# REXJJ/high-fidelity-pointcloud-fusion

Measured on AMD Instinct MI355X. Metric: Mpts/s fused into 1 mm voxel grid, higher is better.
Workload: dtype f64

## Files before the change

### high-fidelity-pointcloud-fusion_amd/csrc/hfpf.hip

```cpp
#include <hip/hip_runtime.h>

#include <cstring>

#include <rocprim/rocprim.hpp>

#include <dlfcn.h>
#include <sched.h>
#include <sys/mman.h>

#if !defined(__HIP_DEVICE_COMPILE__)
#include <emmintrin.h>
#endif
#include <algorithm>
#include <atomic>
#include <condition_variable>
#include <cmath>
#include <cstdarg>
#include <cstdio>
#include <cstdlib>
#include <cstring>
#include <mutex>
#include <string>
#include <thread>
#include <vector>
// ... 109 lines not shown
                    spins = 0;
                }
            }
            if (stop_.load(std::memory_order_acquire)) return;
            seen = g;
            part(i);
            remaining_.fetch_sub(1, std::memory_order_acq_rel);
        }
    }
    std::vector<std::thread> th_;
    std::mutex m_;
    std::condition_variable cv_;
    std::atomic<uint64_t> gen_{0};
    std::atomic<int> remaining_{0}, sleepers_{0};
    std::atomic<bool> stop_{false};
    char* dst_ = nullptr;
    const char* src_ = nullptr;
    size_t bytes_ = 0;
};

constexpr int kStageSlots = 8;
constexpr size_t kXferChunk = 16u << 20;
#ifndef HFPF_PROBE_FRAMES
#define HFPF_PROBE_FRAMES 8
#endif
constexpr int kProbeFrames = HFPF_PROBE_FRAMES;
constexpr int kFrameSlots = 8;

struct DepthSpec {
    uint32_t width, height, depth_f32, depth_step, color_bpp, color_bgr, color_step;
    float cx, cy, sx, sy, unit;
    uint32_t color_off;
    size_t depth_bytes() const { return (size_t)(height - 1) * depth_step + (size_t)width * (depth_f32 ? 4u : 2u); }
    size_t color_bytes() const { return color_bpp ? (size_t)(height - 1) * color_step + (size_t)width * color_bpp : 0; }
};
static_assert(sizeof(DepthSpec) == 13 * 4, "DepthSpec is compared bytewise");

DepthLayout depth_layout(const DepthSpec& d, const void* dev_color, uint64_t color_stride)
{
    return DepthLayout{d.color_bpp ? (const uint8_t*)dev_color : nullptr, color_stride, d.width, d.depth_step, d.color_step, d.depth_f32,
                       d.color_bpp, d.color_bgr, d.cx, d.cy, d.sx, d.sy, d.unit};
}

struct Knobs {
    int copy_streams = 2;
    bool update_cells = true;
    int host_batch = 4;
    int upd_shape_forced = -1;
    bool trace_shape = false;
    bool bin_spare = true;
    bool stream_replay = true;
    float bin_slack = 2.0f;
    bool clean_small_nowait = true;
    float test_bin_scale = 1.f;
    bool test_table_skip = false;
    bool mailbox = true;
    int test_dev_tile = kDevTileDefault;
    int stage_threads = 0;
};

struct Session {
    bool dirty = false;
    uint64_t n_linked[kLogRegions] = {0};
    uint64_t gate_done = 0;
    bool pend_valid = false;
    uint64_t direct_linked = 0;
    bool normals_possible = false;
    uint32_t next_frame_id = 0;
    bool poisoned = false;
    std::string poison_msg;
    bool bin_have_hist = false;
    bool bin_from_probe = false;
    double bin_prev_points = 0;
    uint64_t n_bricks_known = 0;
    uint64_t n_bricks_before = 0;
    unsigned long long upd_miss_seen = 0, upd_member_seen = 0;
    unsigned long long pub_seq = 0;
    uint32_t pend_n = 0, pend_first = 0;
    uint32_t pend_pts = 0;
    uint32_t pend_lay[5] = {0, 0, 0, 0, 0};
    bool pend_depth = false;
    DepthSpec pend_ds{};
    double pend_pose[kFrameSlots * 12] = {0};
    uint64_t occ_exported = 0;
    uint64_t frames_exported = 0, frames_seen = 0;
};

using EventPairs = std::vector<std::pair<hipEvent_t, hipEvent_t>>;

}

struct hfpf_handle {
    std::mutex mtx;
    std::string err;

    hfpf_config cfg;
    GridParams g;
    Knobs knobs;
    bool binned = false;
    int integrate_grid = 1536;
    size_t dir_entries = 0;
    uint64_t n_slots = 0;
    uint64_t max_touched = 0;

    Session ss;
    uint64_t frames_integrated = 0;
    uint64_t clean_passes = 0;
    uint32_t launch_seq = 0;
    bool upd_wide = false;
    bool epoch_used = false;
    unsigned long long mbox_seq = 0;
    int stage_next = 0, fslot_next = 0;

    Tables t;
    hipStream_t stream = nullptr;
    hipStream_t copy_stream = nullptr;
    hipStream_t copy_more[3] = {nullptr, nullptr, nullptr};
    std::vector<void*> allocs;
    uint64_t device_bytes = 0;
    unsigned long long* h_ctr = nullptr;
    unsigned long long* h_log_ctr = nullptr;
    unsigned long long* mbox = nullptr;
    DevBuf pend_a, pend_b;
    StageSlot stage[kStageSlots];
    FrameSlot fslot[kFrameSlots];
    void* ring_d = nullptr;
    size_t ring_cap = 0;
    hipEvent_t busy_ev = nullptr;
    bool busy_pending = false;
    void* xfer_pin[2] = {nullptr, nullptr};
    hipEvent_t xfer_ev[2] = {nullptr, nullptr};
    StagePool* stage_pool = nullptr;
    DevBuf sort_tmp, keys_a, keys_b, vals_a, vals_b, rows_dev, probe_a, probe_b, probe_c, probe_d, probe_e, probe_f;
    DevBuf zbuf, render_pose, render_out;
    DevBuf track_in, track_acc;
    DevBuf query_in, query_out;
    DevBuf mesh_cube, mesh_corner, mesh_kdata, mesh_cdata, mesh_out, mesh_ctr;
    DevBuf comp_index, comp_rows, comp_recs, comp_out;
    DevBuf dev_mesh, dev_tri, dev_bins, dev_pairs, dev_out;
    DevBuf ray_in, ray_out, ray_map;
    DevBuf snap_stage, snap_err;
    uint64_t bin_pool = 0;
    DevBuf bin_pt_buf, bin_rgb_buf, bin_sums;
    DevBuf ovf_pt_buf, ovf_aux_buf;
    bool dist_on = false;
    int rank = 0, world = 1;
    void* rccl_lib = nullptr;
    void* comm = nullptr;
    uint64_t ex_cap_records = 0;
    DevBuf ex_send, ex_recv, ex_counts, stats_total;
    unsigned long long* h_counts = nullptr;

    bool timing = false;
    bool timing_detail = false;
    std::vector<hipEvent_t> ev_detail;
    std::vector<uint8_t> ev_detail_ran;
    double t_detail_ms[3] = {0, 0, 0};
    uint64_t n_detail[3] = {0, 0, 0};
    EventPairs ev_pending, ev_pending_clean;
    EventPairs ev_pending_ray;
// ... 150 lines not shown
    h->h_ctr[C_REPLAY_MEMBER] = replayed;
    unsigned long long upd_tested = 0, upd_member = 0;
    for (int r = 0; r < kLogRegions; r++) {
        upd_tested += h->h_log_ctr[r * 16 + 2];
        upd_member += h->h_log_ctr[r * 16 + 3];
    }
    h->h_ctr[C_DEP_TESTED] += upd_tested;
    h->h_ctr[C_DEP_MEMBER] += upd_member;
    unsigned long long single = 0;
    for (int r = 0; r < kLogRegions; r++) single += h->h_log_ctr[r * 16 + 4];
    h->h_ctr[C_TOUCHED_SINGLE] = single;
    {
        const uint64_t nbk = std::min<uint64_t>(h->h_ctr[C_BRICKS], h->t.max_bricks);
        if (nbk != h->ss.n_bricks_known) h->ss.n_bricks_before = h->ss.n_bricks_known;
        h->ss.n_bricks_known = nbk;
    }
    return HFPF_OK;
}

int check_device_errors(hfpf_handle* h)
{
    const unsigned long long e = h->h_ctr[C_ERR];
    if (!e) return HFPF_OK;
    std::string what;
    if (e & E_BRICKS) what += " brick pool (max_bricks)";
    if (e & E_LOG) what += " point log (max_log_points)";
    if (e & E_OCC) what += " occupied list (max_normals*4)";
    if (e & E_NORMALS) what += " normal records (max_normals)";
    if (e & E_REG) what += " registrations (max_normals*7)";
    if (e & E_DEP) what += " dependant table";
    if (e & E_SPIN) what += " brick-claim spin bound";
    if (e & E_DEPCNT) what += " more than 65535 dependants on one cell";
    if (e & E_FRAME) what += " frame id >= max_frames";
    if (e & E_OVF) what += " integrate overflow list";
    if (e & E_CHAIN) what += " point-log chain / run record out of range (internal)";
    return fail(h, HFPF_ERR_CAPACITY, "device pool overflow:%s", what.c_str());
}

float stat_scale_for(double bound) { return (float)std::ldexp(1.0, 26 - (int)std::floor(std::log2(bound))); }

Knobs read_knobs()
{
    Knobs k;
    if (const char* cs = getenv("HFPF_COPY_STREAMS")) k.copy_streams = std::max(1, std::min(atoi(cs), 4));
    const char* uf = getenv("HFPF_UPDATE_FORM");
    k.update_cells = !(uf && uf[0] == 'p');
    if (const char* hb = getenv("HFPF_HOST_BATCH")) k.host_batch = std::max(1, std::min(atoi(hb), kFrameSlots));
    if (const char* us = getenv("HFPF_UPD_SHAPE")) k.upd_shape_forced = std::max(0, std::min(atoi(us), 1));
    if (const char* tr = getenv("HFPF_TRACE_SHAPE")) k.trace_shape = tr[0] != '0';
    if (const char* sp = getenv("HFPF_BIN_SPARE")) k.bin_spare = sp[0] != '0';
    if (const char* sr = getenv("HFPF_STREAM_REPLAY")) k.stream_replay = sr[0] != '0';
    if (const char* bs = getenv("HFPF_BIN_SLACK")) k.bin_slack = std::max(1.0f, std::min(4.0f, (float)atof(bs)));
    if (const char* nw = getenv("HFPF_CLEAN_NOWAIT")) k.clean_small_nowait = nw[0] != '0';
    if (const char* bs = getenv("HFPF_TEST_BIN_SCALE")) k.test_bin_scale = std::max(0.f, std::min(1.f, (float)atof(bs)));
    const char* ts = getenv("HFPF_TEST_TABLE_SKIP");
    k.test_table_skip = ts && ts[0] == '1';
    if (const char* dt = getenv("HFPF_TEST_DEV_TILE")) k.test_dev_tile = std::max(8, std::min(atoi(dt), kDevTileMax));
    const char* mb = getenv("HFPF_MAILBOX");
    k.mailbox = !mb || mb[0] != '0';
    int cores = (int)std::thread::hardware_concurrency();
    cpu_set_t set;
    if (sched_getaffinity(0, sizeof set, &set) == 0) cores = std::min(cores > 0 ? cores : 1 << 20, CPU_COUNT(&set));
    const char* st = getenv("HFPF_STAGE_THREADS");
    k.stage_threads = st ? std::max(0, std::min(atoi(st), 15)) : std::max(0, std::min(7, cores / 2 - 1));
    return k;
}

int setup_params(hfpf_handle* h)
{
    const hfpf_config& c = h->cfg;
    GridParams& g = h->g;
    if (!(c.resolution > 0.f)) return fail(h, HFPF_ERR_BAD_CONFIG, "resolution must be > 0");
    for (int a = 0; a < 3; a++)
        if (!(c.bbox[2 * a + 1] > c.bbox[2 * a])) return fail(h, HFPF_ERR_BAD_CONFIG, "bounding_box axis %d: max <= min", a);
    if (c.k != 2) return fail(h, HFPF_ERR_BAD_CONFIG, "k must be 2 (the reference probes exactly 125 neighbours, OccupancyGrid.hpp:334)");
    if (c.K < 0 || c.K > 16) return fail(h, HFPF_ERR_BAD_CONFIG, "K out of range [0,16]");
    if (!(c.cylinder_radius > 0) || !(c.ball_radius > 0)) return fail(h, HFPF_ERR_BAD_CONFIG, "radii must be > 0");
    g.res = (double)c.resolution;
    g.inv_res = 1.0 / g.res;
    for (int a = 0; a < 3; a++) {
        g.min[a] = c.bbox[2 * a];
        g.max[a] = c.bbox[2 * a + 1];
        const double d = (g.max[a] - g.min[a]) / g.res;
        if (!(d < 2097151.0)) return fail(h, HFPF_ERR_BAD_CONFIG, "axis %d: more than 2^21 cells", a);
        g.dim[a] = (int32_t)d;
        g.bdim[a] = (g.dim[a] + 1 + 7) / 8;
    }
    {
        auto bits_for = [](int32_t dim) {
            uint32_t b = 1;
            while ((1ll << b) <= (long long)dim) b++;
            return b;
        };
        g.key_sy = bits_for(g.dim[2]);
        g.key_sx = g.key_sy + bits_for(g.dim[1]);
        g.key_bits = g.key_sx + bits_for(g.dim[0]);
    }
    g.zclip_min = c.z_clip_min;
    g.zclip_max = c.z_clip_max;
    {
        auto float_at_or_above = [](double m) {
            float f = (float)m;
            if ((double)f < m) f = nextafterf(f, INFINITY);
            return f;
        };
        auto float_at_or_below = [](double m) {
// ... 92 lines not shown
    int rc;
#define ALLOC(field, count, ...)                                         \
    if ((rc = dev_alloc(h, &t.field, (count), ##__VA_ARGS__)) != HFPF_OK) return rc;
    ALLOC(dir, h->dir_entries, 0, false);
    ALLOC(brick_lin, t.max_bricks + 1);
    ALLOC(info, h->n_slots, 0, false);
    ALLOC(first_frame, h->n_slots, 0, false);
    ALLOC(buf_head, h->n_slots * kChains, 0, false);
    ALLOC(stat_id, h->n_slots, 0, false);
    ALLOC(pre_dep, h->n_slots, 0, false);
    ALLOC(dep_tmp, h->n_slots, 0, false);
    ALLOC(occ_mask, (t.max_bricks + 1) * 8, 0, false);
    ALLOC(log_pt, t.max_log + 1, 0, false);
    if (c.flags & HFPF_FLAG_FUSE_COLOR) { ALLOC(log_rgb, t.max_log + 1, 0, false); }
    ALLOC(occ_list, t.max_occ, 0, false);
    ALLOC(nv_key, t.max_normals + 1, 0, false);
    ALLOC(nv_slot, t.max_normals + 1, 0, false);
    ALLOC(nv_c, 3 * (t.max_normals + 1), 0, false);
    ALLOC(nv_n, 3 * (t.max_normals + 1), 0, false);
    ALLOC(stats, (t.max_normals + 1) * kStatWords, 0, false);
    t.color = (c.flags & HFPF_FLAG_FUSE_COLOR) ? 1u : 0u;
    t.test_table_skip = h->knobs.test_table_skip ? 1u : 0u;
    ALLOC(nd_mask, (t.max_bricks + 1) * 8 * 2, 0, false);
    ALLOC(reg_occ, t.max_reg, 0, false);
    ALLOC(dep, t.max_dep + t.max_normals + 1, 0, false);
    t.nv_line = reinterpret_cast<float4*>(t.dep + t.max_dep);
    ALLOC(prereg_list, t.max_reg, 0, false);
    ALLOC(touched_list, h->max_touched, 0, false);
    ALLOC(run_start, t.max_bricks + 2, 0, false);
    ALLOC(run_len, t.max_bricks + 2, 0, false);
    ALLOC(run_cnt, t.max_bricks + 2);
    ALLOC(cand_key, t.max_occ, 0, false);
    ALLOC(frame_vp, 3 * t.max_frames);
    ALLOC(frame_list, t.max_frames, 0, false);
    ALLOC(ctr, C_COUNT);
    ALLOC(log_ctr, kLogRegions * 16);
    ALLOC(bin_fill, 2 * (t.max_bricks + 2));
    ALLOC(bin_off, 2 * (t.max_bricks + 2));
    ALLOC(bin_capb, 2 * (t.max_bricks + 2));
    h->binned = (c.flags & HFPF_FLAG_DIRECT_UPDATE) == 0;
#undef ALLOC
    t.log_region_cap = t.max_log / kLogRegions;
    t.ent_base = t.dep;
    t.ent_dep_first = 0;
    t.ent_nv_first = t.max_dep;
    return reset_state(h);
}

#ifndef HFPF_SORT_BLOCK_ITEMS
#define HFPF_SORT_BLOCK_ITEMS 4
#endif
using sort_config = rocprim::radix_sort_config<rocprim::default_config, rocprim::merge_sort_config<512, 1024, HFPF_SORT_BLOCK_ITEMS>, rocprim::default_config>;

int sort_keys_u64(hfpf_handle* h, uint64_t* in, uint64_t* out, uint64_t n, unsigned bits = 0)
{
    const unsigned kb = bits ? bits : h->g.key_bits;
    size_t bytes = 0;
    HIPCHK(h, rocprim::radix_sort_keys<sort_config>(nullptr, bytes, in, out, (size_t)n, 0, kb, h->stream));
    int rc = scratch(h, h->sort_tmp, bytes);
    if (rc) return rc;
    bytes = h->sort_tmp.bytes;
    HIPCHK(h, rocprim::radix_sort_keys<sort_config>(h->sort_tmp.p, bytes, in, out, (size_t)n, 0, kb, h->stream));
    return HFPF_OK;
}

int sort_keys_u32(hfpf_handle* h, uint32_t* in, uint32_t* out, uint64_t n, unsigned bits = 32)
{
    size_t bytes = 0;
    HIPCHK(h, rocprim::radix_sort_keys<sort_config>(nullptr, bytes, in, out, (size_t)n, 0, bits, h->stream));
    int rc = scratch(h, h->sort_tmp, bytes);
    if (rc) return rc;
    bytes = h->sort_tmp.bytes;
    HIPCHK(h, rocprim::radix_sort_keys<sort_config>(h->sort_tmp.p, bytes, in, out, (size_t)n, 0, bits, h->stream));
    return HFPF_OK;
}

int sort_pairs_u64(hfpf_handle* h, uint64_t* kin, uint64_t* kout, uint32_t* vin, uint32_t* vout, uint64_t n, unsigned bits = 0)
{
    const unsigned kb = bits ? bits : h->g.key_bits;
    size_t bytes = 0;
    HIPCHK(h, rocprim::radix_sort_pairs<sort_config>(nullptr, bytes, kin, kout, vin, vout, (size_t)n, 0, kb, h->stream));
    int rc = scratch(h, h->sort_tmp, bytes);
    if (rc) return rc;
    bytes = h->sort_tmp.bytes;
    HIPCHK(h, rocprim::radix_sort_pairs<sort_config>(h->sort_tmp.p, bytes, kin, kout, vin, vout, (size_t)n, 0, kb, h->stream));
    return HFPF_OK;
}

int acquire_stage(hfpf_handle* h, uint32_t n_frames, StageSlot** out)
{
    StageSlot& s = h->stage[h->stage_next];
    h->stage_next = (h->stage_next + 1) % kStageSlots;
    if (s.pending) {
        HIPCHK(h, hipEventSynchronize(s.done));
        s.pending = false;
    }
    if (!s.done) HIPCHK(h, hipEventCreateWithFlags(&s.done, hipEventDisableTiming));
    if (s.cap < n_frames) {
        if (s.h_pose) {
            HIPCHK(h, hipHostFree(s.h_pose));
            HIPCHK(h, hipFree(s.d_pose));
            s.h_pose = nullptr, s.d_pose = nullptr, s.cap = 0;
        }
        const uint32_t cap = std::max<uint32_t>(n_frames, 64);
        const size_t bytes = (size_t)cap * (12 * sizeof(double) + sizeof(uint32_t));
        HIPCHK(h, hipHostMalloc((void**)&s.h_pose, bytes, hipHostMallocDefault));
        HIPCHK(h, hipMalloc((void**)&s.d_pose, bytes));
        s.cap = cap;
    }
    s.h_ids = reinterpret_cast<uint32_t*>(s.h_pose + 12 * (size_t)n_frames);
    s.d_ids = reinterpret_cast<uint32_t*>(s.d_pose + 12 * (size_t)n_frames);
    *out = &s;
    return HFPF_OK;
}

int pick_update_shape(hfpf_handle* h, double points, uint32_t nb)
{
    (void)points;
    (void)nb;
    if (h->knobs.upd_shape_forced >= 0) return h->knobs.upd_shape_forced;
    const unsigned long long miss = h->h_ctr[C_TABLE_MISS], member = h->h_ctr[C_DEP_MEMBER] + h->h_ctr[C_REPLAY_MEMBER];
    if (h->knobs.trace_shape)
        fprintf(stderr, "hfpf: update shape window: %llu table misses, %llu members (%llu of them replayed so far), %s\n", miss - std::min(miss, h->ss.upd_miss_seen),
                member - std::min(member, h->ss.upd_member_seen), h->h_ctr[C_REPLAY_MEMBER], h->upd_wide ? "wide" : "dense");
    if (!h->upd_wide && miss > h->ss.upd_miss_seen && (miss - h->ss.upd_miss_seen) * 500ull > member - std::min(member, h->ss.upd_member_seen)) h->upd_wide = true;
    h->ss.upd_miss_seen = miss;
    h->ss.upd_member_seen = member;
    return h->upd_wide ? 1 : 0;
// ... 3736 lines not shown
    PROBE_DOWN(proj_out, h->probe_d, n * 12);
    PROBE_DOWN(dist_out, h->probe_e, n * 8);
    PROBE_DOWN(member_out, h->probe_f, n);
    HIPCHK(h, hipStreamSynchronize(h->stream));
    return HFPF_OK;
}

int hfpf_probe_depth(hfpf_handle* h, const hfpf_depth_image* desc, const void* depth, const void* color, float* xyz_out, uint32_t* rgb_out)
{
    if (!h || !xyz_out || !rgb_out) return HFPF_ERR_BAD_ARG;
    std::lock_guard<std::mutex> lk(h->mtx);
    HIPCHK(h, hipSetDevice(h->cfg.device));
    DepthSpec ds;
    int rc = depth_spec(h, desc, depth, color, &ds);
    if (rc) return rc;
    const uint32_t n = ds.width * ds.height;
    PROBE_UP(h->probe_a, depth, ds.depth_bytes());
    if (ds.color_bpp) {
        PROBE_UP(h->probe_b, color, ds.color_bytes());
    }
    if ((rc = scratch(h, h->probe_c, (size_t)n * 12))) return rc;
    if ((rc = scratch(h, h->probe_d, (size_t)n * 4))) return rc;
    hipLaunchKernelGGL(k_probe_depth, dim3(blocks_for(n, 256)), dim3(256), 0, h->stream, depth_layout(ds, h->probe_b.p, 0), (const uint8_t*)h->probe_a.p, n,
                       (float*)h->probe_c.p, (uint32_t*)h->probe_d.p);
    HIPCHK(h, hipGetLastError());
    PROBE_DOWN(xyz_out, h->probe_c, (size_t)n * 12);
    PROBE_DOWN(rgb_out, h->probe_d, (size_t)n * 4);
    HIPCHK(h, hipStreamSynchronize(h->stream));
    return HFPF_OK;
}

int hfpf_probe_trig(hfpf_handle* h, uint64_t n, const float* y, const float* x, float* atan2_out, float* cos_out, float* sin_out)
{
    if (!h || !y || !x || !atan2_out || !cos_out || !sin_out) return HFPF_ERR_BAD_ARG;
    std::lock_guard<std::mutex> lk(h->mtx);
    HIPCHK(h, hipSetDevice(h->cfg.device));
    if (n == 0) return HFPF_OK;
    int rc;
    PROBE_UP(h->probe_a, y, n * 4);
    PROBE_UP(h->probe_b, x, n * 4);
    if ((rc = scratch(h, h->probe_c, n * 4))) return rc;
    if ((rc = scratch(h, h->probe_d, n * 4))) return rc;
    if ((rc = scratch(h, h->probe_e, n * 4))) return rc;
    hipLaunchKernelGGL(k_probe_trig, dim3(blocks_for(n, 256)), dim3(256), 0, h->stream, n, (const float*)h->probe_a.p, (const float*)h->probe_b.p,
                       (float*)h->probe_c.p, (float*)h->probe_d.p, (float*)h->probe_e.p);
    HIPCHK(h, hipGetLastError());
    PROBE_DOWN(atan2_out, h->probe_c, n * 4);
    PROBE_DOWN(cos_out, h->probe_d, n * 4);
    PROBE_DOWN(sin_out, h->probe_e, n * 4);
    HIPCHK(h, hipStreamSynchronize(h->stream));
    return HFPF_OK;
}

}
```

### high-fidelity-pointcloud-fusion_amd/csrc/kernels.hpp

```cpp
#pragma once
#include <type_traits>

#include "stats.hpp"

namespace hfpf {

typedef float vf4 __attribute__((ext_vector_type(4)));

struct FrameLayout {
    uint32_t point_step, off_x, off_y, off_z, off_rgb;
};

struct DepthLayout {
    const uint8_t* color;
    uint64_t color_stride;
    uint32_t width, depth_step, color_step;
    uint32_t depth_f32;
    uint32_t color_bpp;
    uint32_t color_bgr;
    float cx, cy, sx, sy, unit;
};

template <bool WANT_RGB>
__device__ __forceinline__ vf4 depth_fetch(const uint8_t* __restrict__ dimg, const uint8_t* __restrict__ cimg, const DepthLayout& L, uint32_t i)
// ... 3591 lines not shown
            for (uint32_t e = threadIdx.x; e < nt * 12u; e += 256u) s_tri[e] = ((const double*)recs)[(uint64_t)s_idx[e / 12u] * 12u + e % 12u];
            __syncthreads();
            if (have) {
                for (uint32_t j = 0; j < nt; j++) {
                    double Q[3];
                    uint32_t region;
                    const double dd = dev_closest(P, &s_tri[j * 12u], Q, region);
                    if (dd <= md2 && (!found || dd < best)) {
                        const double* N = &s_tri[j * 12u + 9u];
                        const double rr[3] = {P[0] - Q[0], P[1] - Q[1], P[2] - Q[2]};
                        found = true, best = dd, btri = s_idx[j], breg = region, neg = dev_dot(N, rr) < 0.0;
                        bq[0] = Q[0], bq[1] = Q[1], bq[2] = Q[2];
                    }
                }
            }
        }
        if (have) {
            Deviation d;
            if (found) {
                d.distance = (float)sqrt(best);
                d.signed_distance = neg ? -d.distance : d.distance;
                d.tri = btri, d.flags = kDevFound | breg;
                d.q[0] = (float)bq[0], d.q[1] = (float)bq[1], d.q[2] = (float)bq[2];
                const double w = (double)d.distance;
                n_found++;
                n_neg += d.signed_distance < 0.f ? 1u : 0u;
                max_bits = max(max_bits, __float_as_uint(d.distance));
                sum_abs += llrint(w * 0x1p30);
                sum_sq += llrint((w * w) * 0x1p30);
            } else {
                d.distance = d.signed_distance = d.q[0] = d.q[1] = d.q[2] = __uint_as_float(0x7FC00000u);
                d.tri = 0xFFFFFFFFu, d.flags = 0u;
            }
            d.reserved = 0u;
            out[row] = d;
        }
    }
    for (int o = 32; o > 0; o >>= 1) {
        n_found += __shfl_down(n_found, o);
        n_neg += __shfl_down(n_neg, o);
        sum_abs += __shfl_down(sum_abs, o);
        sum_sq += __shfl_down(sum_sq, o);
        max_bits = max(max_bits, __shfl_down(max_bits, o));
    }
    if ((threadIdx.x & 63u) == 0 && n_found) {
        atomicAdd(&sum->n_found, n_found);
        if (n_neg) atomicAdd(&sum->n_negative, n_neg);
        atomicAdd((unsigned long long*)&sum->sum_abs_q30, (unsigned long long)sum_abs);
        atomicAdd((unsigned long long*)&sum->sum_sq_q30, (unsigned long long)sum_sq);
        atomicMax(&sum->max_abs_bits, max_bits);
    }
}

}
```

### high-fidelity-pointcloud-fusion_amd/python/hfpf.py

```python
import ctypes as C
import os
import subprocess

import numpy as np

_HERE = os.path.dirname(os.path.abspath(__file__))
PKG_DIR = os.path.dirname(_HERE)
CSRC_DIR = os.path.join(PKG_DIR, "csrc")
LIB_PATH = os.environ.get("HFPF_LIB") or os.path.join(CSRC_DIR, "libhfpf.so")

FLAG_FUSE_COLOR = 1
FLAG_PCL_SHIFTED_COV = 2
FLAG_DIRECT_UPDATE = 4
STATUS = {0: "OK", -1: "BAD_CONFIG", -2: "BAD_ARG", -3: "CAPACITY", -4: "HIP", -5: "STATE", -6: "IO", -7: "DIST"}


class HfpfError(RuntimeError):
    def __init__(self, code, msg):
        super().__init__("hfpf status %d (%s): %s" % (code, STATUS.get(code, "?"), msg))
        self.code = code


class Config(C.Structure):
    _fields_ = [
        ("struct_size", C.c_uint32),
        ("resolution", C.c_float),
        ("bbox", C.c_double * 6),
        ("k", C.c_int32),
        ("K", C.c_int32),
        ("gate", C.c_int32),
        ("cylinder_radius", C.c_double),
        ("ball_radius", C.c_double),
        ("z_clip_min", C.c_double),
        ("z_clip_max", C.c_double),
        ("device", C.c_int32),
        ("flags", C.c_uint32),
        ("max_bricks", C.c_uint64),
        ("max_log_points", C.c_uint64),
        ("max_normals", C.c_uint64),
        ("max_frames", C.c_uint64),
        ("frame_width", C.c_uint32),
        ("reserved0", C.c_uint32),
        ("max_call_points", C.c_uint64),
    ]


class ExtractOpts(C.Structure):
    _fields_ = [("struct_size", C.c_uint32), ("classify_threshold", C.c_int32), ("min_count", C.c_double),
                ("paint_white", C.c_int32), ("reserved0", C.c_int32)]


class Counters(C.Structure):
    _fields_ = [(n, C.c_uint64) for n in (
        "points_presented", "points_zclip_pass", "points_in_bbox", "points_buffered", "dep_pairs_tested",
        "dep_pairs_member", "voxels_occupied", "voxels_with_normal", "bricks_allocated", "registrations",
        "dep_entries", "frames_integrated", "clean_passes", "device_bytes", "replay_members", "points_direct", "table_misses", "update_extra_rounds")]


ROW_DTYPE = np.dtype(
    [
        ("ix", "<i4"), ("iy", "<i4"), ("iz", "<i4"), ("count", "<u4"),
        ("x", "<f4"), ("y", "<f4"), ("z", "<f4"),
        ("nx", "<f4"), ("ny", "<f4"), ("nz", "<f4"),
        ("sdx", "<f4"), ("sdy", "<f4"), ("sdz", "<f4"),
        ("mean_dist", "<f4"), ("sd_dist", "<f4"), ("rgb", "<u4"),
    ]
)

EXPORTS = [
    "hfpf_default_config", "hfpf_abi_version", "hfpf_create", "hfpf_destroy", "hfpf_last_error", "hfpf_get_dims",
    "hfpf_integrate", "hfpf_integrate_pinned", "hfpf_host_alloc", "hfpf_host_free", "hfpf_integrate_device", "hfpf_is_dirty", "hfpf_clean", "hfpf_extract", "hfpf_extract_filtered", "hfpf_free_rows",
    "hfpf_write_pcd", "hfpf_write_meta_csv", "hfpf_write_pcd_xyzrgb", "hfpf_write_pcd_binary", "hfpf_clear", "hfpf_sync", "hfpf_get_counters", "hfpf_get_occupied",
    "hfpf_device_alloc", "hfpf_device_free", "hfpf_device_upload", "hfpf_kernel_timing", "hfpf_get_kernel_time",
    "hfpf_probe_points", "hfpf_probe_normals", "hfpf_probe_project", "hfpf_probe_trig",
    "hfpf_dist_unique_id", "hfpf_dist_init", "hfpf_dist_info", "hfpf_dist_disable", "hfpf_epoch_export", "hfpf_epoch_import", "hfpf_stats_export",
    "hfpf_extract_with_stats", "hfpf_device_download", "hfpf_device_copy", "hfpf_epoch_import_gathered",
    "hfpf_integrate_depth", "hfpf_integrate_depth_pinned", "hfpf_integrate_depth_device", "hfpf_probe_depth",
    "hfpf_render", "hfpf_render_device",
    "hfpf_track_depth", "hfpf_track_depth_device", "hfpf_track",
    "hfpf_query", "hfpf_query_device", "hfpf_query_depth",
    "hfpf_extract_mesh", "hfpf_extract_mesh_device", "hfpf_free_mesh", "hfpf_write_ply", "hfpf_check_mesh_opts",
    "hfpf_check_component_opts", "hfpf_extract_components", "hfpf_extract_components_device", "hfpf_free_components",
    "hfpf_check_deviation_opts", "hfpf_compare_mesh", "hfpf_compare_mesh_device", "hfpf_free_deviation", "hfpf_read_ply",
    "hfpf_check_raycast_opts", "hfpf_raycast", "hfpf_raycast_device", "hfpf_raycast_view", "hfpf_raycast_view_device",
    "hfpf_snapshot", "hfpf_free_snapshot", "hfpf_restore", "hfpf_save", "hfpf_load", "hfpf_snapshot_info", "hfpf_config_from_snapshot",
]

DEPTH_U16, DEPTH_F32 = 1, 2
COLOR_NONE, COLOR_RGB8, COLOR_BGR8, COLOR_RGBA8, COLOR_BGRA8 = 0, 1, 2, 3, 4
COLOR_BPP = {COLOR_NONE: 0, COLOR_RGB8: 3, COLOR_BGR8: 3, COLOR_RGBA8: 4, COLOR_BGRA8: 4}


class DepthImage(C.Structure):
    _fields_ = [("struct_size", C.c_uint32), ("width", C.c_uint32), ("height", C.c_uint32), ("depth_format", C.c_uint32),
                ("depth_step", C.c_uint32), ("depth_scale", C.c_float), ("fx", C.c_double), ("fy", C.c_double),
                ("cx", C.c_double), ("cy", C.c_double), ("color_format", C.c_uint32), ("color_step", C.c_uint32),
                ("reserved", C.c_uint64)]


def depth_desc(width, height, depth_format, depth_step, K, color_format=COLOR_NONE, color_step=0, depth_scale=0.001):
    d = DepthImage()
    d.struct_size = C.sizeof(DepthImage)
    d.width, d.height, d.depth_format, d.depth_step = width, height, depth_format, depth_step
    d.depth_scale = depth_scale
    d.fx, d.fy, d.cx, d.cy = (float(k) for k in K)
    d.color_format, d.color_step = color_format, color_step
    return d


def _image_desc(depth, K, color, color_format, depth_scale):
    if depth.ndim != 2 or depth.dtype not in (np.uint16, np.float32) or depth.strides[1] != depth.itemsize:
        raise ValueError("depth must be a 2-D uint16 or float32 image with contiguous rows")
    fmt = DEPTH_U16 if depth.dtype == np.uint16 else DEPTH_F32
    H, W = depth.shape
    cstep = 0
    if color is None:
        color_format = COLOR_NONE
    else:
        if color.dtype != np.uint8 or color.ndim != 3 or color.shape[:2] != depth.shape or color.strides[2] != 1 or color.strides[1] != color.shape[2]:
            raise ValueError("color must be a HxWx3 or HxWx4 uint8 image with contiguous rows, the size of the depth image")
        if color_format is None:
            color_format = COLOR_RGB8 if color.shape[2] == 3 else COLOR_RGBA8
        if COLOR_BPP.get(color_format) != color.shape[2]:
            raise ValueError("color_format %r does not match a %d-channel image" % (color_format, color.shape[2]))
        cstep = color.strides[0]
    return depth_desc(W, H, fmt, depth.strides[0], K, color_format, cstep, depth_scale)

RENDER_CULL_BACKFACES = 1
RENDER_WORLD_NORMALS = 2
RENDER_PLANES = (("depth", np.float32, 1), ("normal", np.float32, 3), ("rgb", np.uint32, 1), ("count", np.uint32, 1), ("voxel", np.int32, 3))
# ... 304 lines not shown
    L = C.CDLL(LIB_PATH)
    vp, u32, u64, i32 = C.c_void_p, C.c_uint32, C.c_uint64, C.c_int32
    L.hfpf_default_config.argtypes = [C.POINTER(Config)]
    L.hfpf_default_config.restype = None
    L.hfpf_abi_version.restype = C.c_int
    L.hfpf_create.argtypes = [C.POINTER(Config), C.POINTER(vp)]
    L.hfpf_destroy.argtypes = [vp]
    L.hfpf_last_error.argtypes = [vp]
    L.hfpf_last_error.restype = C.c_char_p
    L.hfpf_get_dims.argtypes = [vp, C.POINTER(i32), C.POINTER(C.c_double)]
    L.hfpf_integrate.argtypes = [vp, vp, u32, u32, u32, u32, u32, u32, vp]
    L.hfpf_integrate_device.argtypes = [vp, vp, u32, u64, u32, u32, u32, u32, u32, u32, vp, vp]
    L.hfpf_integrate_pinned.argtypes = [vp, vp, u32, u32, u32, u32, u32, u32, vp]
    L.hfpf_host_alloc.argtypes = [vp, u64, C.POINTER(vp)]
    L.hfpf_host_free.argtypes = [vp, vp]
    L.hfpf_is_dirty.argtypes = [vp]
    L.hfpf_clean.argtypes = [vp]
    L.hfpf_extract.argtypes = [vp, C.POINTER(vp), C.POINTER(u64)]
    L.hfpf_extract_filtered.argtypes = [vp, C.POINTER(ExtractOpts), C.POINTER(vp), C.POINTER(u64)]
    L.hfpf_free_rows.argtypes = [vp]
    L.hfpf_free_rows.restype = None
    L.hfpf_write_pcd.argtypes = [vp, u64, C.c_char_p]
    L.hfpf_write_meta_csv.argtypes = [vp, u64, C.c_char_p]
    L.hfpf_write_pcd_xyzrgb.argtypes = [vp, u64, C.c_char_p, u32, i32, i32]
    L.hfpf_write_pcd_binary.argtypes = [vp, u64, C.c_char_p]
    L.hfpf_clear.argtypes = [vp]
    L.hfpf_sync.argtypes = [vp]
    L.hfpf_get_counters.argtypes = [vp, C.POINTER(Counters)]
    L.hfpf_get_occupied.argtypes = [vp, vp, u64, C.POINTER(u64)]
    L.hfpf_device_alloc.argtypes = [vp, u64, C.POINTER(vp)]
    L.hfpf_device_free.argtypes = [vp, vp]
    L.hfpf_device_upload.argtypes = [vp, vp, vp, u64]
    L.hfpf_kernel_timing.argtypes = [vp, C.c_int]
    L.hfpf_get_kernel_time.argtypes = [vp, C.c_int, C.POINTER(C.c_double), C.POINTER(u64)]
    L.hfpf_probe_points.argtypes = [vp, vp, vp, u64, vp, vp, vp]
    L.hfpf_probe_normals.argtypes = [vp, u64, vp, vp, vp, vp, vp]
    L.hfpf_probe_project.argtypes = [vp, u64, vp, vp, vp, vp, vp, vp]
    L.hfpf_probe_trig.argtypes = [vp, u64, vp, vp, vp, vp, vp]
    L.hfpf_dist_unique_id.argtypes = [vp]
    L.hfpf_dist_init.argtypes = [vp, C.c_int, C.c_int, vp]
    L.hfpf_dist_disable.argtypes = [vp]
    L.hfpf_dist_info.argtypes = [vp, C.POINTER(i32), C.POINTER(i32)]
    L.hfpf_epoch_export.argtypes = [vp, C.POINTER(vp), C.POINTER(u64)]
    L.hfpf_epoch_import.argtypes = [vp, vp, u64]
    L.hfpf_stats_export.argtypes = [vp, C.POINTER(vp), C.POINTER(u64), C.POINTER(vp), C.POINTER(u64)]
    L.hfpf_extract_with_stats.argtypes = [vp, vp, vp, C.POINTER(vp), C.POINTER(u64)]
    L.hfpf_device_download.argtypes = [vp, vp, vp, u64]
    L.hfpf_device_copy.argtypes = [vp, vp, vp, u64]
    L.hfpf_epoch_import_gathered.argtypes = [vp, vp, u64, i32, i32, vp]
    L.hfpf_integrate_depth.argtypes = [vp, C.POINTER(DepthImage), vp, vp, vp]
    L.hfpf_integrate_depth_pinned.argtypes = [vp, C.POINTER(DepthImage), vp, vp, vp]
    L.hfpf_integrate_depth_device.argtypes = [vp, C.POINTER(DepthImage), vp, u64, vp, u64, u32, vp, vp]
    L.hfpf_probe_depth.argtypes = [vp, C.POINTER(DepthImage), vp, vp, vp, vp]
    L.hfpf_render.argtypes = [vp, C.POINTER(RenderOpts), vp, C.POINTER(RenderPlanes)]
    L.hfpf_render_device.argtypes = [vp, C.POINTER(RenderOpts), u32, vp, C.POINTER(RenderPlanes)]
    L.hfpf_track_depth.argtypes = [vp, C.POINTER(TrackOpts), C.POINTER(DepthImage), vp, vp, C.POINTER(TrackResult)]
    L.hfpf_track_depth_device.argtypes = [vp, C.POINTER(TrackOpts), C.POINTER(DepthImage), vp, vp, C.POINTER(TrackResult)]
    L.hfpf_track.argtypes = [vp, C.POINTER(TrackOpts), vp, u32, u32, u32, u32, u32, vp, C.POINTER(TrackResult)]
    L.hfpf_query.argtypes = [vp, C.POINTER(QueryOpts), vp, u32, u32, u32, u32, u32, vp, vp, vp]
    L.hfpf_query_device.argtypes = [vp, C.POINTER(QueryOpts), vp, u32, u32, u32, u32, u32, vp, vp, vp]
    L.hfpf_query_depth.argtypes = [vp, C.POINTER(QueryOpts), C.POINTER(DepthImage), vp, vp, vp, vp]
    L.hfpf_extract_mesh.argtypes = [vp, C.POINTER(MeshOpts), C.POINTER(vp), C.POINTER(u64), C.POINTER(vp), C.POINTER(u64)]
    L.hfpf_extract_mesh_device.argtypes = [vp, C.POINTER(MeshOpts), C.POINTER(vp), C.POINTER(u64), C.POINTER(vp), C.POINTER(u64)]
    L.hfpf_free_mesh.argtypes = [vp, vp]
    L.hfpf_free_mesh.restype = None
    L.hfpf_write_ply.argtypes = [vp, u64, vp, u64, C.c_char_p]
    L.hfpf_check_mesh_opts.argtypes = [C.POINTER(MeshOpts)]
    L.hfpf_check_component_opts.argtypes = [C.POINTER(ComponentOpts)]
    for fn in (L.hfpf_extract_components, L.hfpf_extract_components_device):
        fn.argtypes = [vp, C.POINTER(ComponentOpts), C.POINTER(vp), C.POINTER(vp), C.POINTER(u64), C.POINTER(vp), C.POINTER(u64)]
    L.hfpf_free_components.argtypes = [vp, vp, vp]
    L.hfpf_free_components.restype = None
    L.hfpf_check_deviation_opts.argtypes = [C.POINTER(DeviationOpts)]
    for fn in (L.hfpf_compare_mesh, L.hfpf_compare_mesh_device):
        fn.argtypes = [vp, C.POINTER(DeviationOpts), vp, u64, u32, vp, u64, vp, C.POINTER(vp), C.POINTER(vp), C.POINTER(u64),
                       C.POINTER(DeviationSummary)]
    L.hfpf_free_deviation.argtypes = [vp, vp]
    L.hfpf_free_deviation.restype = None
    L.hfpf_read_ply.argtypes = [C.c_char_p, C.POINTER(vp), C.POINTER(u64), C.POINTER(vp), C.POINTER(u64)]
    dbl = C.c_double
    L.hfpf_check_raycast_opts.argtypes = [C.POINTER(RaycastOpts)]
    L.hfpf_raycast.argtypes = [vp, C.POINTER(RaycastOpts), vp, u64, vp, vp]
    L.hfpf_raycast_device.argtypes = [vp, C.POINTER(RaycastOpts), vp, u64, vp, vp]
    L.hfpf_raycast_view.argtypes = [vp, C.POINTER(RaycastOpts), u32, u32, dbl, dbl, dbl, dbl, vp, vp]
    L.hfpf_raycast_view_device.argtypes = [vp, C.POINTER(RaycastOpts), u32, u32, dbl, dbl, dbl, dbl, u32, vp, vp]
    L.hfpf_snapshot.argtypes = [vp, C.POINTER(vp), C.POINTER(u64)]
    L.hfpf_free_snapshot.argtypes = [vp]
    L.hfpf_free_snapshot.restype = None
    L.hfpf_restore.argtypes = [vp, vp, u64]
    L.hfpf_save.argtypes = [vp, C.c_char_p]
    L.hfpf_load.argtypes = [vp, C.c_char_p]
    L.hfpf_snapshot_info.argtypes = [vp, u64, C.POINTER(SnapshotInfo)]
    L.hfpf_config_from_snapshot.argtypes = [C.POINTER(SnapshotInfo), C.POINTER(Config)]
    _lib = L
    return L


def _p(a):
    return a.ctypes.data_as(C.c_void_p)


def default_config():
    c = Config()
    lib().hfpf_default_config(C.byref(c))
    return c

# ... 502 lines not shown
        return ms.value, n.value

    def probe_points(self, pose, xyz):
        pose = np.ascontiguousarray(pose, dtype=np.float64).reshape(12)
        xyz = np.ascontiguousarray(xyz, dtype=np.float32).reshape(-1, 3)
        n = xyz.shape[0]
        q = np.zeros((n, 3), np.float32)
        idx = np.zeros((n, 3), np.int32)
        flags = np.zeros(n, np.uint8)
        self._chk(lib().hfpf_probe_points(self._h, _p(pose), _p(xyz), n, _p(q), _p(idx), _p(flags)))
        return q, idx, flags

    def probe_normals(self, cells, occ, vps):
        cells = np.ascontiguousarray(cells, dtype=np.int32).reshape(-1, 3)
        n = cells.shape[0]
        occ = np.ascontiguousarray(occ, dtype=np.uint8).reshape(n, 125)
        vps = np.ascontiguousarray(vps, dtype=np.float32).reshape(n, 3)
        normals = np.zeros((n, 3), np.float32)
        totals = np.zeros(n, np.int32)
        self._chk(lib().hfpf_probe_normals(self._h, n, _p(cells), _p(occ), _p(vps), _p(normals), _p(totals)))
        return normals, totals

    def probe_project(self, pts, centres, normals):
        pts = np.ascontiguousarray(pts, dtype=np.float32).reshape(-1, 3)
        n = pts.shape[0]
        centres = np.ascontiguousarray(centres, dtype=np.float32).reshape(n, 3)
        normals = np.ascontiguousarray(normals, dtype=np.float32).reshape(n, 3)
        proj = np.zeros((n, 3), np.float32)
        dist = np.zeros(n, np.float64)
        member = np.zeros(n, np.uint8)
        self._chk(lib().hfpf_probe_project(self._h, n, _p(pts), _p(centres), _p(normals), _p(proj), _p(dist), _p(member)))
        self.last_member_kernel_form = (member & 2) != 0
        self.last_hoisted_division_same = (member & 4) != 0
        return proj, dist, (member & 1) != 0

    def probe_depth(self, depth, K, color=None, color_format=None, depth_scale=0.001):
        d = _image_desc(depth, K, color, color_format, depth_scale)
        n = d.width * d.height
        xyz = np.zeros((n, 3), np.float32)
        rgb = np.zeros(n, np.uint32)
        self._chk(lib().hfpf_probe_depth(self._h, C.byref(d), C.c_void_p(depth.ctypes.data),
                                         C.c_void_p(color.ctypes.data) if color is not None else None, _p(xyz), _p(rgb)))
        return xyz, rgb

    def probe_trig(self, y, x):
        y = np.ascontiguousarray(y, dtype=np.float32)
        x = np.ascontiguousarray(x, dtype=np.float32)
        a = np.zeros_like(x)
        c = np.zeros_like(x)
        s = np.zeros_like(x)
        self._chk(lib().hfpf_probe_trig(self._h, x.size, _p(y), _p(x), _p(a), _p(c), _p(s)))
        return a, c, s


def dist_unique_id():
    buf = (C.c_char * 128)()
    rc = lib().hfpf_dist_unique_id(buf)
    if rc != 0:
        raise HfpfError(rc, lib().hfpf_last_error(None).decode())
    return bytes(buf)


def write_pcd(rows, path):
    rows = np.ascontiguousarray(rows, dtype=ROW_DTYPE)
    rc = lib().hfpf_write_pcd(_p(rows), rows.size, os.fsencode(path))
    if rc != 0:
        raise HfpfError(rc, "write_pcd(%s)" % path)


def write_meta_csv(rows, path):
    rows = np.ascontiguousarray(rows, dtype=ROW_DTYPE)
    rc = lib().hfpf_write_meta_csv(_p(rows), rows.size, os.fsencode(path))
    if rc != 0:
        raise HfpfError(rc, "write_meta_csv(%s)" % path)


def write_pcd_xyzrgb(rows, path, min_count=0, classify_threshold=-1, white=True):
    rows = np.ascontiguousarray(rows, dtype=ROW_DTYPE)
    rc = lib().hfpf_write_pcd_xyzrgb(_p(rows), rows.size, os.fsencode(path), min_count, classify_threshold, 1 if white else 0)
    if rc != 0:
        raise HfpfError(rc, "write_pcd_xyzrgb(%s)" % path)


def write_pcd_binary(rows, path):
    rows = np.ascontiguousarray(rows, dtype=ROW_DTYPE)
    rc = lib().hfpf_write_pcd_binary(_p(rows), rows.size, os.fsencode(path))
    if rc != 0:
        raise HfpfError(rc, "write_pcd_binary(%s)" % path)
```

### include/hfpf_probe.h

```cpp
#ifndef HFPF_PROBE_H
#define HFPF_PROBE_H
#include "hfpf.h"
#ifdef __cplusplus
extern "C" {
#endif

int hfpf_probe_points(hfpf_handle* h, const double pose_3x4[12], const float* xyz, uint64_t n, float* q_out,
                      int32_t* idx_out, uint8_t* flags_out);
int hfpf_probe_normals(hfpf_handle* h, uint64_t n, const int32_t* cells, const uint8_t* occ, const float* vps,
                       float* normals_out, int32_t* totals_out);
int hfpf_probe_project(hfpf_handle* h, uint64_t n, const float* pts, const float* centres, const float* normals,
                       float* proj_out, double* dist_out, uint8_t* member_out);
int hfpf_probe_depth(hfpf_handle* h, const hfpf_depth_image* desc, const void* depth, const void* color, float* xyz_out,
                     uint32_t* rgb_out);
int hfpf_probe_trig(hfpf_handle* h, uint64_t n, const float* y, const float* x, float* atan2_out, float* cos_out,
                    float* sin_out);

#ifdef __cplusplus
}
#endif
#endif
```

Measured before the change: 28240.

## Add single-block LDS radix sort for small key arrays

Adds a one-workgroup, 1024-thread radix sort kernel, using 5-bit digits with shared-memory counters. sort_keys_u32 and sort_keys_u64 now route arrays of up to about 31.7K keys to it instead of rocprim's multi-launch radix sort. The aim is to cut launch count, scratch-size queries and temporary buffer use on the many small sorts. It also adds a probe entry point for testing. The risk is that a single block is slower than rocprim for inputs near the size cap or with many key bits.

Result: no change. 28230 (-0.0%).

```diff
diff --git a/high-fidelity-pointcloud-fusion_amd/csrc/hfpf.hip b/high-fidelity-pointcloud-fusion_amd/csrc/hfpf.hip
--- a/high-fidelity-pointcloud-fusion_amd/csrc/hfpf.hip
+++ b/high-fidelity-pointcloud-fusion_amd/csrc/hfpf.hip
@@ -185,6 +185,7 @@
     bool stream_replay = true;
     float bin_slack = 2.0f;
     bool clean_small_nowait = true;
+    bool sort_small = true;
     float test_bin_scale = 1.f;
     bool test_table_skip = false;
     bool mailbox = true;
@@ -239,6 +240,7 @@
     Session ss;
     uint64_t frames_integrated = 0;
     uint64_t clean_passes = 0;
+    uint64_t sort_small_launches = 0;
     uint32_t launch_seq = 0;
     bool upd_wide = false;
     bool epoch_used = false;
@@ -495,6 +497,7 @@
     if (const char* sr = getenv("HFPF_STREAM_REPLAY")) k.stream_replay = sr[0] != '0';
     if (const char* bs = getenv("HFPF_BIN_SLACK")) k.bin_slack = std::max(1.0f, std::min(4.0f, (float)atof(bs)));
     if (const char* nw = getenv("HFPF_CLEAN_NOWAIT")) k.clean_small_nowait = nw[0] != '0';
+    if (const char* ss = getenv("HFPF_SORT_SMALL")) k.sort_small = ss[0] != '0';
     if (const char* bs = getenv("HFPF_TEST_BIN_SCALE")) k.test_bin_scale = std::max(0.f, std::min(1.f, (float)atof(bs)));
     const char* ts = getenv("HFPF_TEST_TABLE_SKIP");
     k.test_table_skip = ts && ts[0] == '1';
@@ -693,20 +696,27 @@
 #endif
 using sort_config = rocprim::radix_sort_config<rocprim::default_config, rocprim::merge_sort_config<512, 1024, HFPF_SORT_BLOCK_ITEMS>, rocprim::default_config>;
 
-int sort_keys_u64(hfpf_handle* h, uint64_t* in, uint64_t* out, uint64_t n, unsigned bits = 0)
-{
-    const unsigned kb = bits ? bits : h->g.key_bits;
-    size_t bytes = 0;
-    HIPCHK(h, rocprim::radix_sort_keys<sort_config>(nullptr, bytes, in, out, (size_t)n, 0, kb, h->stream));
-    int rc = scratch(h, h->sort_tmp, bytes);
-    if (rc) return rc;
-    bytes = h->sort_tmp.bytes;
-    HIPCHK(h, rocprim::radix_sort_keys<sort_config>(h->sort_tmp.p, bytes, in, out, (size_t)n, 0, kb, h->stream));
-    return HFPF_OK;
-}
-
-int sort_keys_u32(hfpf_handle* h, uint32_t* in, uint32_t* out, uint64_t n, unsigned bits = 32)
-{
+template <typename K>
+int sort_small(hfpf_handle* h, const K* in, K* out, uint32_t n, unsigned bits)
+{
+    const uint32_t ipt = (n + kSortSmallThreads - 1) / kSortSmallThreads;
+#define HFPF_SORT_SMALL_LAUNCH(I) hipLaunchKernelGGL((k_sort_small<K, I>), dim3(1), dim3(kSortSmallThreads), 0, h->stream, in, out, n, (uint32_t)bits)
+    if (ipt <= 5) HFPF_SORT_SMALL_LAUNCH(5);
+    else if (ipt <= 13) HFPF_SORT_SMALL_LAUNCH(13);
+    else if (ipt <= 21) HFPF_SORT_SMALL_LAUNCH(21);
+    else if (ipt <= 27) HFPF_SORT_SMALL_LAUNCH(27);
+    else HFPF_SORT_SMALL_LAUNCH(kSortSmallItems);
+#undef HFPF_SORT_SMALL_LAUNCH
+    HIPCHK(h, hipGetLastError());
+    h->sort_small_launches++;
+    return HFPF_OK;
+}
+
+template <typename K>
+int sort_keys(hfpf_handle* h, K* in, K* out, uint64_t n, unsigned bits)
+{
+    if (n == 0) return HFPF_OK;
+    if (n <= kSortSmallMax && h->knobs.sort_small) return sort_small<K>(h, in, out, (uint32_t)n, bits);
     size_t bytes = 0;
     HIPCHK(h, rocprim::radix_sort_keys<sort_config>(nullptr, bytes, in, out, (size_t)n, 0, bits, h->stream));
     int rc = scratch(h, h->sort_tmp, bytes);
@@ -715,6 +725,10 @@
     HIPCHK(h, rocprim::radix_sort_keys<sort_config>(h->sort_tmp.p, bytes, in, out, (size_t)n, 0, bits, h->stream));
     return HFPF_OK;
 }
+
+int sort_keys_u64(hfpf_handle* h, uint64_t* in, uint64_t* out, uint64_t n, unsigned bits = 0) { return sort_keys<uint64_t>(h, in, out, n, bits ? bits : h->g.key_bits); }
+
+int sort_keys_u32(hfpf_handle* h, uint32_t* in, uint32_t* out, uint64_t n, unsigned bits = 32) { return sort_keys<uint32_t>(h, in, out, n, bits); }
 
 int sort_pairs_u64(hfpf_handle* h, uint64_t* kin, uint64_t* kout, uint32_t* vin, uint32_t* vout, uint64_t n, unsigned bits = 0)
 {
@@ -4557,4 +4571,25 @@
     return HFPF_OK;
 }
 
-}
+int hfpf_probe_sort(hfpf_handle* h, uint32_t key_bytes, uint32_t bits, uint64_t n, const void* keys, uint64_t n_buf, void* buf, int32_t* used_small)
+{
+    if (!h || !keys || !buf || !used_small || (key_bytes != 4 && key_bytes != 8) || bits < 1 || bits > 8 * key_bytes || n_buf < n || n_buf > (1ull << 28))
+        return HFPF_ERR_BAD_ARG;
+    std::lock_guard<std::mutex> lk(h->mtx);
+    HIPCHK(h, hipSetDevice(h->cfg.device));
+    *used_small = 0;
+    if (n == 0) return HFPF_OK;
+    int rc;
+    PROBE_UP(h->probe_a, keys, n * key_bytes);
+    PROBE_UP(h->probe_b, buf, n_buf * key_bytes);
+    const uint64_t before = h->sort_small_launches;
+    if (key_bytes == 8) rc = sort_keys_u64(h, (uint64_t*)h->probe_a.p, (uint64_t*)h->probe_b.p, n, bits);
+    else rc = sort_keys_u32(h, (uint32_t*)h->probe_a.p, (uint32_t*)h->probe_b.p, n, bits);
+    if (rc) return rc;
+    *used_small = h->sort_small_launches != before;
+    PROBE_DOWN(buf, h->probe_b, n_buf * key_bytes);
+    HIPCHK(h, hipStreamSynchronize(h->stream));
+    return HFPF_OK;
+}
+
+}
diff --git a/high-fidelity-pointcloud-fusion_amd/csrc/kernels.hpp b/high-fidelity-pointcloud-fusion_amd/csrc/kernels.hpp
--- a/high-fidelity-pointcloud-fusion_amd/csrc/kernels.hpp
+++ b/high-fidelity-pointcloud-fusion_amd/csrc/kernels.hpp
@@ -3667,4 +3667,138 @@
     }
 }
 
-}
+constexpr int kSortSmallThreads = 1024;
+constexpr int kSortSmallItems = 31;
+constexpr uint32_t kSortSmallMax = (uint32_t)kSortSmallThreads * kSortSmallItems;
+constexpr int kSortSmallDigit = 5;
+constexpr int kSortSmallBins = 1 << kSortSmallDigit;
+
+template <int IPT, bool TO_STRIPED>
+__device__ __forceinline__ void sort_small_exchange(uint32_t* s_x, uint32_t (&v)[IPT], const uint32_t* pos, uint32_t t)
+{
+#pragma unroll
+    for (int i = 0; i < IPT; i++) {
+        s_x[pos ? (pos[i >> 1] >> (16 * (i & 1))) & 0xFFFFu : (uint32_t)i * kSortSmallThreads + t] = v[i];
+        __builtin_amdgcn_sched_barrier(0);
+    }
+    __syncthreads();
+#pragma unroll
+    for (int i = 0; i < IPT; i++) v[i] = TO_STRIPED ? s_x[(uint32_t)i * kSortSmallThreads + t] : s_x[t * IPT + i];
+    __syncthreads();
+}
+
+template <typename K, int IPT>
+__global__ __launch_bounds__(kSortSmallThreads) void k_sort_small(const K* __restrict__ in, K* __restrict__ out, uint32_t n, uint32_t bits)
+{
+    constexpr uint32_t T = kSortSmallThreads;
+    constexpr bool WIDE = sizeof(K) == 8;
+    constexpr uint32_t kCntWords = kSortSmallBins * T / 2;
+    constexpr uint32_t kWords = IPT * T > kCntWords ? IPT * T : kCntWords;
+    static_assert(IPT >= 1 && IPT <= kSortSmallItems && (IPT & 1), "odd, at most kSortSmallItems");
+    static_assert(kSortSmallBins == 32 && IPT * T < 65536, "a thread scans 32 counters; a prefix fits 16 bits");
+    __shared__ __attribute__((aligned(16))) uint32_t s_x[kWords];
+    __shared__ uint32_t s_wsum[T / 64];
+    uint16_t* s_cnt = (uint16_t*)s_x;
+    const uint32_t t = threadIdx.x;
+
+    uint32_t lo[IPT], hi[WIDE ? IPT : 1];
+    uint32_t rank[(IPT + 1) / 2];
+#pragma unroll
+    for (int i = 0; i < IPT; i++) {
+        const uint32_t p = (uint32_t)i * T + t;
+        K k = ~(K)0;
+        if (p < n) k = in[p];
+        lo[i] = (uint32_t)k;
+        if constexpr (WIDE) hi[i] = (uint32_t)((uint64_t)k >> 32);
+    }
+    sort_small_exchange<IPT, false>(s_x, lo, nullptr, t);
+    if constexpr (WIDE) sort_small_exchange<IPT, false>(s_x, hi, nullptr, t);
+
+    const uint32_t passes = (bits + kSortSmallDigit - 1) / kSortSmallDigit;
+    for (uint32_t pass = 0; pass < passes; pass++) {
+        const uint32_t shift = pass * kSortSmallDigit;
+        const uint32_t mask = (1u << min((uint32_t)kSortSmallDigit, bits - shift)) - 1u;
+        auto digit = [&](int i, uint32_t shift) -> uint32_t {
+            uint32_t w;
+            if constexpr (WIDE) w = (uint32_t)((((uint64_t)hi[i] << 32) | lo[i]) >> shift);
+            else w = lo[i] >> shift;
+            return w & mask;
+        };
+#pragma unroll
+        for (uint32_t j = 0; j < kCntWords / T; j++) s_x[j * T + t] = 0u;
+        __syncthreads();
+#pragma unroll
+        for (int i = 0; i < IPT; i++) {
+            const uint32_t c = digit(i, shift) * T + t;
+            const uint32_t before = s_cnt[c];
+            rank[i >> 1] = (i & 1) ? rank[i >> 1] | (before << 16) : before;
+            asm volatile("" : "+v"(rank[i >> 1]));
+            s_cnt[c] = (uint16_t)(before + 1u);
+            __builtin_amdgcn_sched_barrier(0);
+        }
+        __syncthreads();
+        {
+            uint32_t total = 0;
+#pragma unroll
+            for (int j = 0; j < 4; j++) {
+                const uint4 q = ((const uint4*)s_x)[t * 4 + j];
+                total += (q.x & 0xFFFFu) + (q.x >> 16) + (q.y & 0xFFFFu) + (q.y >> 16) + (q.z & 0xFFFFu) + (q.z >> 16) + (q.w & 0xFFFFu) + (q.w >> 16);
+            }
+            uint32_t incl = total;
+#pragma unroll
+            for (uint32_t d = 1; d < 64; d <<= 1) {
+                const uint32_t up = __shfl_up(incl, d);
+                if ((t & 63u) >= d) incl += up;
+            }
+            if ((t & 63u) == 63u) s_wsum[t >> 6] = incl;
+            __syncthreads();
+            uint32_t run = incl - total;
+            for (uint32_t wv = 0; wv < (t >> 6); wv++) run += s_wsum[wv];
+            auto prefix = [&](uint32_t w) -> uint32_t {
+                const uint32_t a = w & 0xFFFFu, b = w >> 16;
+                const uint32_t r = run | ((run + a) << 16);
+                run += a + b;
+                return r;
+            };
+#pragma unroll
+            for (int j = 0; j < 4; j++) {
+                uint4 q = ((const uint4*)s_x)[t * 4 + j];
+                q.x = prefix(q.x), q.y = prefix(q.y), q.z = prefix(q.z), q.w = prefix(q.w);
+                ((uint4*)s_x)[t * 4 + j] = q;
+            }
+        }
+        __syncthreads();
+        uint32_t shift_again = shift;
+        asm volatile("" : "+s"(shift_again));
+#pragma unroll
+        for (int i = 0; i < IPT; i++) {
+            rank[i >> 1] += (uint32_t)s_cnt[digit(i, shift_again) * T + t] << (16 * (i & 1));
+            __builtin_amdgcn_sched_barrier(0);
+        }
+        __syncthreads();
+        if (pass + 1 < passes) {
+            sort_small_exchange<IPT, false>(s_x, lo, rank, t);
+            if constexpr (WIDE) sort_small_exchange<IPT, false>(s_x, hi, rank, t);
+        } else {
+            sort_small_exchange<IPT, true>(s_x, lo, rank, t);
+            if constexpr (WIDE) sort_small_exchange<IPT, true>(s_x, hi, rank, t);
+        }
+    }
+    if (passes == 0) {
+        uint32_t self[(IPT + 1) / 2];
+#pragma unroll
+        for (int i = 0; i < IPT; i++) self[i >> 1] = (i & 1) ? self[i >> 1] | ((t * IPT + i) << 16) : t * IPT + i;
+        sort_small_exchange<IPT, true>(s_x, lo, self, t);
+        if constexpr (WIDE) sort_small_exchange<IPT, true>(s_x, hi, self, t);
+    }
+#pragma unroll
+    for (int i = 0; i < IPT; i++) {
+        const uint32_t p = (uint32_t)i * T + t;
+        if (p < n) {
+            if constexpr (WIDE) out[p] = (K)(((uint64_t)hi[i] << 32) | lo[i]);
+            else out[p] = (K)lo[i];
+        }
+    }
+}
+
+}
diff --git a/high-fidelity-pointcloud-fusion_amd/python/hfpf.py b/high-fidelity-pointcloud-fusion_amd/python/hfpf.py
--- a/high-fidelity-pointcloud-fusion_amd/python/hfpf.py
+++ b/high-fidelity-pointcloud-fusion_amd/python/hfpf.py
@@ -75,7 +75,7 @@
     "hfpf_probe_points", "hfpf_probe_normals", "hfpf_probe_project", "hfpf_probe_trig",
     "hfpf_dist_unique_id", "hfpf_dist_init", "hfpf_dist_info", "hfpf_dist_disable", "hfpf_epoch_export", "hfpf_epoch_import", "hfpf_stats_export",
     "hfpf_extract_with_stats", "hfpf_device_download", "hfpf_device_copy", "hfpf_epoch_import_gathered",
-    "hfpf_integrate_depth", "hfpf_integrate_depth_pinned", "hfpf_integrate_depth_device", "hfpf_probe_depth",
+    "hfpf_integrate_depth", "hfpf_integrate_depth_pinned", "hfpf_integrate_depth_device", "hfpf_probe_depth", "hfpf_probe_sort",
     "hfpf_render", "hfpf_render_device",
     "hfpf_track_depth", "hfpf_track_depth_device", "hfpf_track",
     "hfpf_query", "hfpf_query_device", "hfpf_query_depth",
@@ -486,6 +486,7 @@
     L.hfpf_integrate_depth_pinned.argtypes = [vp, C.POINTER(DepthImage), vp, vp, vp]
     L.hfpf_integrate_depth_device.argtypes = [vp, C.POINTER(DepthImage), vp, u64, vp, u64, u32, vp, vp]
     L.hfpf_probe_depth.argtypes = [vp, C.POINTER(DepthImage), vp, vp, vp, vp]
+    L.hfpf_probe_sort.argtypes = [vp, C.c_uint32, C.c_uint32, u64, vp, u64, vp, vp]
     L.hfpf_render.argtypes = [vp, C.POINTER(RenderOpts), vp, C.POINTER(RenderPlanes)]
     L.hfpf_render_device.argtypes = [vp, C.POINTER(RenderOpts), u32, vp, C.POINTER(RenderPlanes)]
     L.hfpf_track_depth.argtypes = [vp, C.POINTER(TrackOpts), C.POINTER(DepthImage), vp, vp, C.POINTER(TrackResult)]
@@ -1094,6 +1095,14 @@
         self._chk(lib().hfpf_probe_trig(self._h, x.size, _p(y), _p(x), _p(a), _p(c), _p(s)))
         return a, c, s
 
+    def probe_sort(self, keys, bits, guard=0, fill=0):
+        keys = np.ascontiguousarray(keys)
+        assert keys.dtype in (np.uint32, np.uint64) and keys.ndim == 1
+        buf = np.full(keys.size + guard, fill, keys.dtype)
+        small = C.c_int32(0)
+        self._chk(lib().hfpf_probe_sort(self._h, keys.dtype.itemsize, bits, keys.size, _p(keys), buf.size, _p(buf), C.byref(small)))
+        return buf, bool(small.value)
+
 
 def dist_unique_id():
     buf = (C.c_char * 128)()
diff --git a/include/hfpf_probe.h b/include/hfpf_probe.h
--- a/include/hfpf_probe.h
+++ b/include/hfpf_probe.h
@@ -15,6 +15,8 @@
                      uint32_t* rgb_out);
 int hfpf_probe_trig(hfpf_handle* h, uint64_t n, const float* y, const float* x, float* atan2_out, float* cos_out,
                     float* sin_out);
+int hfpf_probe_sort(hfpf_handle* h, uint32_t key_bytes, uint32_t bits, uint64_t n, const void* keys, uint64_t n_buf, void* buf,
+                    int32_t* used_small);
 
 #ifdef __cplusplus
 }
```
